# fulliu/lc

Measured on AMD Instinct MI355X. Metric: poses/sec (cov-loss fwd+bwd + weighted PnP), B=256 N=64, 1/2/4/8 MI355X, higher is better.
Workload: dtype f64; 1 GPU; configs[1]: synthetic B=256 N=64 2D-3D correspondences per GPU, HIP weighted-PnP + cov-loss; global_batch=256, n_points=64, launch=graph_region, launch_agreed_by_all_ranks=True

## Files before the change

### lc_amd/csrc/lc_common.h

```cpp
#pragma once
#include <hip/hip_runtime.h>

#include "shared/lc_shared.h"

namespace lc {

typedef float lc_v4f_t __attribute__((ext_vector_type(4)));
__device__ __forceinline__ void store_stream4(float* q, float a, float b, float c, float d) {
    lc_v4f_t r = {a, b, c, d};
    __builtin_nontemporal_store(r, reinterpret_cast<lc_v4f_t*>(q));
}


__device__ __forceinline__ double fast_rcp(double x) {
    const double y = __builtin_amdgcn_rcp(x);
    const double e = __builtin_fma(-x, y, 1.0);
    return __builtin_fma(y, e, y);
}

__device__ __forceinline__ void fast_sqrt_rsqrt(double x, double& s, double& rs) {
    const double r0 = __builtin_amdgcn_rsq(x);
    const double g = x * r0, h = 0.5 * r0;
    const double rr = __builtin_fma(-h, g, 0.5);
    const double g1 = __builtin_fma(g, rr, g), h1 = __builtin_fma(h, rr, h);
    s = x == 0.0 ? 0.0 : g1;
    rs = x == 0.0 ? r0 : 2.0 * h1;
}
__device__ __forceinline__ double fast_sqrt(double x) {
    double s, rs;
    fast_sqrt_rsqrt(x, s, rs);
    return s;
}

__device__ __forceinline__ void wave_sync() {
    __builtin_amdgcn_fence(__ATOMIC_RELEASE, "wavefront");
    __builtin_amdgcn_wave_barrier();
    __builtin_amdgcn_fence(__ATOMIC_ACQUIRE, "wavefront");
}

constexpr int block_sum_lds_doubles(int K) { return K * 68 + K; }
__device__ __forceinline__ int block_sum_open(int lane) {
    wave_sync();
    return lane + 2 * (lane >> 5);
}
template <int ROW = 68>
__device__ __forceinline__ void block_sum_put(double* lds, int pos, int k, double v) { lds[k * ROW + pos] = v; }

__device__ __forceinline__ double block_sum_segment(const double2* row) {
    double2 a[8];
#pragma unroll
    for (int i = 0; i < 8; ++i) a[i] = row[i];
#pragma unroll
    for (int i = 0; i < 8; ++i) {
        const double2 t = row[8 + i];
        a[i].x += t.x;
        a[i].y += t.y;
    }
#pragma unroll
    for (int st = 4; st >= 1; st >>= 1) {
#pragma unroll
        for (int i = 0; i < st; ++i) { a[i].x += a[i + st].x; a[i].y += a[i + st].y; }
    }
    return a[0].x + a[0].y;
}
__device__ __forceinline__ double block_sum_segment_component(const double* d) {
    double a[8];
#pragma unroll
    for (int i = 0; i < 8; ++i) a[i] = d[2 * i];
#pragma unroll
    for (int i = 0; i < 8; ++i) a[i] += d[16 + 2 * i];
#pragma unroll
    for (int st = 4; st >= 1; st >>= 1) {
#pragma unroll
        for (int i = 0; i < st; ++i) a[i] += a[i + st];
    }
    return a[0];
}

template <int K>
__device__ __forceinline__ void block_sum_close(double (&v)[K], double* lds, int lane) {
    static_assert(K <= 32, "two segments per entry, one lane each");
    wave_sync();
    double s = 0;
    if (lane < 2 * K) s = block_sum_segment(reinterpret_cast<const double2*>(lds + (lane / 2) * 68 + 34 * (lane % 2)));
    s += dpp_mov_f64<kDppQuadXor1>(s, s);
    double* tot = lds + K * 68;
    if (lane < 2 * K && (lane % 2) == 0) tot[lane / 2] = s;
    wave_sync();
#pragma unroll
    for (int k = 0; k < K; ++k) v[k] = tot[k];
}

template <class T>
__device__ __forceinline__ void xcd_store(T* q, T v) { __hip_atomic_store(q, v, __ATOMIC_RELAXED, __HIP_MEMORY_SCOPE_AGENT); }
template <class T>
__device__ __forceinline__ T xcd_load(const T* q) { return __hip_atomic_load(q, __ATOMIC_RELAXED, __HIP_MEMORY_SCOPE_AGENT); }
__device__ __forceinline__ void xcd_stores_done() { asm volatile("s_waitcnt vmcnt(0)" ::: "memory"); }

constexpr int kArrivalShards = 16, kArrivalStride = 32;
constexpr int kArrivalWords = (1 + kArrivalShards) * kArrivalStride;
__device__ __forceinline__ bool arrive_is_last(unsigned* words, unsigned block, unsigned blocks) {
    const unsigned shards = blocks < (unsigned)kArrivalShards ? blocks : (unsigned)kArrivalShards;
    const unsigned g = block % shards, members = (blocks - g + shards - 1) / shards;
    if (__hip_atomic_fetch_add(words + (1 + g) * kArrivalStride, 1u, __ATOMIC_RELAXED, __HIP_MEMORY_SCOPE_AGENT) != members - 1) return false;
    return __hip_atomic_fetch_add(words, 1u, __ATOMIC_RELAXED, __HIP_MEMORY_SCOPE_AGENT) == shards - 1;
}
__device__ __forceinline__ void arrival_reset(unsigned* words, int tid) {
    if (tid <= kArrivalShards) xcd_store(words + tid * kArrivalStride, 0u);
}

constexpr int kTeamRowDoubles = 66;
static_assert(kTeamRowDoubles >= 66 && kTeamRowDoubles % 4 == 2, "a row holds two padded segments; rows of one wave fall on different banks");
constexpr int sum_team2_lds_doubles(int K) { return K * kTeamRowDoubles + 2 * K; }
template <int K, int W>
__device__ __forceinline__ void block_sum_team2(double (&v)[K], double* lds, int lane, int& phase) {
    static_assert(K % 2 == 0 && K <= 32 && (W == 0 || W == 1), "an even number of entries dealt to two waves");
    wave_sync();
    double s = 0;
    const int comp = lane & 1, seg = (lane >> 1) & 1, entry = 2 * (lane >> 2) + W;
    if (lane < 2 * K) s = block_sum_segment_component(lds + entry * kTeamRowDoubles + 34 * seg + comp);
    s += dpp_mov_f64<kDppQuadXor1>(s, s);
    s += dpp_mov_f64<kDppQuadXor2>(s, s);
    double* tot = lds + K * kTeamRowDoubles + K * phase;
    phase ^= 1;
    if (lane < 2 * K && (lane % 4) == 0) tot[entry] = s;
    __syncthreads();
#pragma unroll
    for (int k = 0; k < K; ++k) v[k] = tot[k];
}

template <int K>
__device__ __forceinline__ void block_sum_waves4(double (&v)[K], double* lds, int tid, int& phase) {
    static_assert(K <= 32, "one reduce-scatter of 32");
    const int lane = tid & 63, wave = tid >> 6;
    double w[32];
#pragma unroll
    for (int k = 0; k < 32; ++k) w[k] = k < K ? v[k] : 0.0;
    wave_reduce_scatter16<32>(w, lane);
    double* part = lds;
    double* tot = lds + 128 + 32 * phase;
    phase ^= 1;
    if ((lane & 3) == 0) *reinterpret_cast<double2*>(part + 32 * wave + scatter16_base(lane, 2)) = make_double2(w[0], w[1]);
    __syncthreads();
    if (tid < 32) tot[tid] = ((part[tid] + part[32 + tid]) + part[64 + tid]) + part[96 + tid];
    __syncthreads();
#pragma unroll
    for (int k = 0; k < K; ++k) v[k] = tot[k];
}

constexpr int kSplitMaxParts = 8;
#ifndef LC_SPLIT_WAIT_US
#define LC_SPLIT_WAIT_US 2000
#endif
constexpr unsigned long long kSplitWaitTicks = 100ull * LC_SPLIT_WAIT_US;
__device__ __forceinline__ bool split_wait_expired(int polls, unsigned long long& t0) {
    if ((polls & 15) != 15) return false;
    const unsigned long long now = __builtin_amdgcn_s_memrealtime();
    if (t0 == 0) { t0 = now; return false; }
    return now - t0 > kSplitWaitTicks;
}
constexpr int kSplitRowWords = 64;
constexpr size_t kSplitPoseBytes = 2 * kSplitMaxParts * kSplitRowWords * sizeof(unsigned long long) + 128;
constexpr int kSplitLdsDoubles = 128 + 64 + 2;
constexpr int kSplitSerialLdsDoubles = 128 + 32 * kSplitMaxParts + 32;
struct SplitSum {
    unsigned long long* exch;
    unsigned* epoch;
    int G, part;
    unsigned base;
    unsigned seq;
    bool timed_out;
};
__device__ __forceinline__ unsigned* split_tail(void* region, size_t region_bytes) {
    return reinterpret_cast<unsigned*>(static_cast<char*>(region) + region_bytes - 128);
}
__device__ __forceinline__ SplitSum split_sum_enter(void* pose_region, int G, int part) {
    unsigned* epoch = split_tail(pose_region, kSplitPoseBytes);
    return SplitSum{reinterpret_cast<unsigned long long*>(pose_region), epoch, G, part, xcd_load(epoch), 0u, false};
}
__device__ __forceinline__ void split_sum_leave(const SplitSum& sx) {
    if (sx.timed_out) xcd_store(sx.epoch + 1, 1u);
    else if (sx.part == 0 && sx.seq > 0) xcd_store(sx.epoch, sx.base + sx.seq);
}
__device__ __forceinline__ bool split_rescue_enter(void* region, size_t region_bytes, bool redo, int tid, int threads) {
    unsigned* tail = split_tail(region, region_bytes);
    const bool dirty = xcd_load(tail + 1) != 0u;
    if (!dirty && !redo) return false;
    __syncthreads();
    if (dirty) {
        unsigned long long* w = static_cast<unsigned long long*>(region);
        for (size_t i = tid; i < (region_bytes - 128) / 8; i += threads) xcd_store(w + i, 0ull);
        if (tid < 2) xcd_store(tail + tid, 0u);
    }
    if (redo && tid == 0) xcd_store(tail + 2, xcd_load(tail + 2) + 1u);
    return redo;
}

template <int K>
__device__ __forceinline__ void block_sum_split(double (&v)[K], double* lds, int tid, int& phase, SplitSum& sx) {
    static_assert(K <= 32, "one reduce-scatter of 32");
    const int lane = tid & 63, wave = tid >> 6;
    double w[32];
#pragma unroll
    for (int k = 0; k < 32; ++k) w[k] = k < K ? v[k] : 0.0;
    wave_reduce_scatter16<32>(w, lane);
    double* part = lds;
    double* tot = lds + 128 + 32 * phase;
    int* arrived_ok = reinterpret_cast<int*>(lds + 192);
    phase ^= 1;
    if (sx.timed_out) {
#pragma unroll
        for (int k = 0; k < K; ++k) v[k] = 0.0;
        return;
    }
    if ((lane & 3) == 0) *reinterpret_cast<double2*>(part + 32 * wave + scatter16_base(lane, 2)) = make_double2(w[0], w[1]);
    __syncthreads();
    if (tid < 32) {
        const unsigned long long ticket = (unsigned long long)(sx.base + sx.seq + 1u) << 32;
        unsigned long long* rows = sx.exch + (size_t)(sx.seq & 1u) * (kSplitMaxParts * kSplitRowWords) + 2 * tid;
        {
            const unsigned long long bits = __builtin_bit_cast(unsigned long long, ((part[tid] + part[32 + tid]) + part[64 + tid]) + part[96 + tid]);
            unsigned long long* mine = rows + sx.part * kSplitRowWords;
            xcd_store(mine, ticket | (bits & 0xFFFFFFFFull));
            xcd_store(mine + 1, ticket | (bits >> 32));
        }
        unsigned long long lo[kSplitMaxParts], hi[kSplitMaxParts];
        bool ok = true;
        unsigned long long t0 = 0;
        for (int polls = 0;; ++polls) {
#pragma unroll
            for (int g = 0; g < kSplitMaxParts; ++g)
                if (g < sx.G) {
                    lo[g] = xcd_load(rows + g * kSplitRowWords);
                    hi[g] = xcd_load(rows + g * kSplitRowWords + 1);
                }
            unsigned long long late = 0;
#pragma unroll
            for (int g = 0; g < kSplitMaxParts; ++g)
                if (g < sx.G) late |= ((lo[g] ^ ticket) | (hi[g] ^ ticket)) >> 32;
            if (late == 0) break;
            if (split_wait_expired(polls, t0)) { ok = false; break; }
            __builtin_amdgcn_s_sleep(1);
        }
        double s = 0.0;
#pragma unroll
        for (int g = 0; g < kSplitMaxParts; ++g)
            if (g < sx.G) s += __builtin_bit_cast(double, (hi[g] << 32) | (lo[g] & 0xFFFFFFFFull));
        tot[tid] = s;
        if (!ok) *arrived_ok = 0;
    }
    __syncthreads();
    if (!*arrived_ok) sx.timed_out = true;
#pragma unroll
    for (int k = 0; k < K; ++k) v[k] = tot[k];
    ++sx.seq;
}

template <int K>
__device__ __forceinline__ void block_sum_parts_serial(double (&v)[K], double* lds, int tid, int g, int G) {
    static_assert(K <= 32, "one reduce-scatter of 32");
    const int lane = tid & 63, wave = tid >> 6;
    double w[32];
#pragma unroll
    for (int k = 0; k < 32; ++k) w[k] = k < K ? v[k] : 0.0;
    wave_reduce_scatter16<32>(w, lane);
    double* part = lds;
    double* rows = lds + 128;
    double* tot = lds + 128 + 32 * kSplitMaxParts;
    if ((lane & 3) == 0) *reinterpret_cast<double2*>(part + 32 * wave + scatter16_base(lane, 2)) = make_double2(w[0], w[1]);
    __syncthreads();
    if (tid < 32) {
        rows[32 * g + tid] = ((part[tid] + part[32 + tid]) + part[64 + tid]) + part[96 + tid];
        if (g == G - 1) {
            double s = 0.0;
            for (int h = 0; h < G; ++h) s += rows[32 * h + tid];
            tot[tid] = s;
        }
    }
    __syncthreads();
    if (g == G - 1) {
#pragma unroll
        for (int k = 0; k < K; ++k) v[k] = tot[k];
    }
}

__device__ __forceinline__ double horner_step(double p, double z, double c) {
    double r;
    asm("v_fma_f64 %0, %1, %2, %3" : "=v"(r) : "v"(p), "v"(z), "v"(c));
    return r;
}

#ifndef LC_SINCOS_FALLBACK_CALL
#define LC_SINCOS_FALLBACK_CALL 0
#endif
#if LC_SINCOS_FALLBACK_CALL
static __device__ __attribute__((noinline, cold)) double2 sincos_full_range(double x) {
    double s, c;
    sincos(x, &s, &c);
    return make_double2(s, c);
}
#endif
static __device__ __forceinline__ void sincos_small(double x, double& s, double& c) {
#if LC_SINCOS_FALLBACK_CALL
    if (__builtin_expect(!(x < 1.0e4), 0)) {
        const double2 sc = sincos_full_range(x);
        s = sc.x;
        c = sc.y;
        return;
    }
#else
    if (!(x < 1.0e4)) {
        sincos(x, &s, &c);
        return;
    }
#endif
    const double kf = __builtin_rint(x * 0.63661977236758134308);
    const int q = (int)kf;
    double r = __builtin_fma(-kf, 1.57079632673412561417e+00, x);
    r = __builtin_fma(-kf, 6.07710050650619224932e-11, r);
    r = __builtin_fma(-kf, 2.02226624879595063154e-21, r);
    const double z = r * r;
    double ps = horner_step(1.58969099521155010221e-10, z, -2.50507602534068634195e-08);
    ps = horner_step(ps, z, 2.75573137070700676789e-06);
    ps = horner_step(ps, z, -1.98412698298579493134e-04);
    ps = horner_step(ps, z, 8.33333333332248946124e-03);
    ps = horner_step(ps, z, -1.66666666666666324348e-01);
    const double sr = __builtin_fma(ps * z, r, r);
    double pc = horner_step(-1.13596475577881948265e-11, z, 2.08757232129817482790e-09);
    pc = horner_step(pc, z, -2.75573143513906633035e-07);
    pc = horner_step(pc, z, 2.48015872894767294178e-05);
    pc = horner_step(pc, z, -1.38888888888741095749e-03);
    pc = horner_step(pc, z, 4.16666666666666019037e-02);
    const double cr = __builtin_fma(pc * z, z, __builtin_fma(-0.5, z, 1.0));
    const double ss = (q & 1) ? cr : sr, cc = (q & 1) ? sr : cr;
    s = (q & 2) ? -ss : ss;
    c = ((q + 1) & 2) ? -cc : cc;
}

__device__ __forceinline__ double atan_ratio_pos(double s, double c) {
    const bool swap = s > c;
    const double a = swap ? c : s, b = swap ? s : c;
    double t = a * fast_rcp(b);
#pragma unroll
    for (int k = 0; k < 2; ++k) {
        const double h = fast_sqrt(__builtin_fma(t, t, 1.0));
        t = t * fast_rcp(1.0 + h);
    }
    const double w = t * t;
    double p = horner_step(-1.0 / 21.0, w, 1.0 / 19.0);
    p = horner_step(p, w, -1.0 / 17.0);
    p = horner_step(p, w, 1.0 / 15.0);
    p = horner_step(p, w, -1.0 / 13.0);
    p = horner_step(p, w, 1.0 / 11.0);
    p = horner_step(p, w, -1.0 / 9.0);
    p = horner_step(p, w, 1.0 / 7.0);
    p = horner_step(p, w, -1.0 / 5.0);
    p = horner_step(p, w, 1.0 / 3.0);
    const double at = 4.0 * __builtin_fma(-(p * w), t, t);
    return swap ? 1.57079632679489661923 - at : at;
}

__device__ __forceinline__ bool uniform(bool c) { return __builtin_amdgcn_ballot_w64(c) != 0ull; }

}
```

### lc_amd/csrc/lc_pnp_body.h

```cpp
#pragma once
#include <cfloat>

#include "lc_common.h"
#include "lc_kernels.h"

#ifdef LC_STAMPS
#define LC_PSTAMP_DECL unsigned long long pst_[8] = {0, 0, 0, 0, 0, 0, 0, 0}, pt0_ = 0, pt1_ = 0
#define LC_PSTAMP_BEGIN()                                                                 \
    do {                                                                                  \
        __builtin_amdgcn_sched_barrier(0);                                                \
        asm volatile("s_memtime %0\n\ts_waitcnt lgkmcnt(0)" : "=s"(pt0_)::"memory");      \
        __builtin_amdgcn_sched_barrier(0);                                                \
    } while (0)
#define LC_PSTAMP(i)                                                                      \
    do {                                                                                  \
        __builtin_amdgcn_sched_barrier(0);                                                \
        asm volatile("s_memtime %0\n\ts_waitcnt lgkmcnt(0)" : "=s"(pt1_)::"memory");      \
        __builtin_amdgcn_sched_barrier(0);                                                \
        pst_[i] += pt1_ - pt0_;                                                           \
        pt0_ = pt1_;                                                                      \
    } while (0)
#else
#define LC_PSTAMP_DECL
#define LC_PSTAMP_BEGIN() do {} while (0)
#define LC_PSTAMP(i) do {} while (0)
#endif

#ifndef LC_PNP_TEAM2
#define LC_PNP_TEAM2 1
#endif

namespace lc {
namespace pnp {

template <int NW>
constexpr int kPnpLdsDoubles = [] { static_assert(NW == 1, "the four-wave kernels: kPnpWideReservedLdsDoubles"); return block_sum_lds_doubles(28); }();
constexpr int kPnpTeamLdsDoubles = sum_team2_lds_doubles(28);
constexpr int kPnpWideReservedLdsDoubles = 28 * 68 * 4 + 28;
static_assert(kPnpWideReservedLdsDoubles == 7644 && kPnpWideReservedLdsDoubles >= 128 + 64, "reserved size kept; block_sum_waves4 fits");

struct Point {
    double X[3];
    double u, v;
    double a, b, c;
};

struct Rot {
    double R[9];
    double Jr[9];
};

__device__ __forceinline__ void make_rot(const double aa[3], Rot& o) {
    const double x = aa[0], y = aa[1], z = aa[2];
    const double th2 = x * x + y * y + z * z;
    const bool small = !(th2 > DBL_EPSILON);
    double th, ith;
    fast_sqrt_rsqrt(th2, th, ith);
    double s, c;
    sincos_small(th, s, c);
    const double ith2 = ith * ith;
    const double A = small ? 1.0 : s * ith;
    const double B = small ? 0.0 : (1.0 - c) * ith2;
    const double C = small ? 0.0 : (th - s) * ith2 * ith;
    const double cd = small ? 1.0 : c;
    o.R[0] = cd + B * x * x;    o.R[1] = B * x * y - A * z; o.R[2] = B * x * z + A * y;
    o.R[3] = B * x * y + A * z; o.R[4] = cd + B * y * y;    o.R[5] = B * y * z - A * x;
    o.R[6] = B * x * z - A * y; o.R[7] = B * y * z + A * x; o.R[8] = cd + B * z * z;
    const double d = 1.0 - C * th2;
    o.Jr[0] = d + C * x * x;     o.Jr[1] = C * x * y + B * z; o.Jr[2] = C * x * z - B * y;
    o.Jr[3] = C * x * y - B * z; o.Jr[4] = d + C * y * y;     o.Jr[5] = C * y * z + B * x;
    o.Jr[6] = C * x * z + B * y; o.Jr[7] = C * y * z - B * x; o.Jr[8] = d + C * z * z;
}

template <bool FIRST, bool STREAM = false, int PAR = -1>
__device__ __forceinline__ void accumulate_point(const Point& pt, const Rot& rt, const double t[3], const double k[6],
                                                 const double (&sc)[6], double (&acc)[28], double* lds = nullptr, int pos = 0) {
    double rx[3], q[3];
#pragma unroll
    for (int d = 0; d < 3; ++d) {
        rx[d] = rt.R[3 * d] * pt.X[0] + rt.R[3 * d + 1] * pt.X[1] + rt.R[3 * d + 2] * pt.X[2];
        q[d] = rx[d] + t[d];
    }
    const double iz = fast_rcp(q[2]);
    const double up = (q[0] * k[0] + q[1] * k[1]) * iz, vp = (q[0] * k[3] + q[1] * k[4]) * iz;
    const double du = up - pt.u, dv = vp - pt.v;
    const double r[2] = {du * pt.a + dv * pt.b, dv * pt.c};
    const double dup[3] = {k[0] * iz, k[1] * iz, -up * iz};
    const double dvp[3] = {k[3] * iz, k[4] * iz, -vp * iz};
    double J[2][6];
#pragma unroll
    for (int m = 0; m < 3; ++m) {
        J[0][3 + m] = pt.a * dup[m] + pt.b * dvp[m];
        J[1][3 + m] = pt.c * dvp[m];
    }
#pragma unroll
    for (int rr = 0; rr < 2; ++rr) {
        double cr[3];
        cr[0] = rx[1] * J[rr][5] - rx[2] * J[rr][4];
        cr[1] = rx[2] * J[rr][3] - rx[0] * J[rr][5];
        cr[2] = rx[0] * J[rr][4] - rx[1] * J[rr][3];
#pragma unroll
        for (int m = 0; m < 3; ++m) J[rr][m] = (rt.Jr[3 * m] * cr[0] + rt.Jr[3 * m + 1] * cr[1] + rt.Jr[3 * m + 2] * cr[2]) * sc[m];
#pragma unroll
        for (int m = 0; m < 3; ++m) J[rr][3 + m] *= sc[3 + m];
    }
    static_assert(PAR < 0 || STREAM, "entries are dealt by parity where they go to their LDS slots");
    constexpr auto mine = [](int k) { return PAR < 0 || (k & 1) == PAR; };
    constexpr int kRow = PAR < 0 ? 68 : kTeamRowDoubles;
#pragma unroll
    for (int i = 0; i < 6; ++i) {
#pragma unroll
        for (int j = i; j < 6; ++j) {
            if (mine(tri6(i, j))) {
                const double v = __builtin_fma(J[0][i], J[0][j], J[1][i] * J[1][j]);
                if constexpr (STREAM) block_sum_put<kRow>(lds, pos, tri6(i, j), v);
                else acc[tri6(i, j)] = FIRST ? v : acc[tri6(i, j)] + v;
            }
        }
        if (mine(21 + i)) {
            const double gi = __builtin_fma(J[0][i], r[0], J[1][i] * r[1]);
            if constexpr (STREAM) block_sum_put<kRow>(lds, pos, 21 + i, gi);
            else acc[21 + i] = FIRST ? gi : acc[21 + i] + gi;
        }
    }
    if (mine(27)) {
        const double ss = __builtin_fma(r[0], r[0], r[1] * r[1]);
        if constexpr (STREAM) block_sum_put<kRow>(lds, pos, 27, ss);
        else acc[27] = FIRST ? ss : acc[27] + ss;
    }
}

__device__ __forceinline__ bool ldlt_solve6(const double (&A)[21], const double (&dg)[6], const double (&rhs)[6], double (&y)[6]) {
    double L[6][6], Ld[6][6], id[6];
    bool ok = true;
#pragma unroll
    for (int j = 0; j < 6; ++j) {
        double dj = A[tri6(j, j)] + dg[j];
#pragma unroll
        for (int k = 0; k < j; ++k) dj -= L[j][k] * Ld[j][k];
        ok = ok && (dj > 0) && (dj < DBL_MAX);
        id[j] = fast_rcp(dj);
#pragma unroll
        for (int i = j + 1; i < 6; ++i) {
            double v = A[tri6(j, i)];
#pragma unroll
            for (int k = 0; k < j; ++k) v -= L[i][k] * Ld[j][k];
            Ld[i][j] = v;
            L[i][j] = v * id[j];
        }
    }
    double z[6];
#pragma unroll
    for (int i = 0; i < 6; ++i) {
        double v = rhs[i];
#pragma unroll
        for (int k = 0; k < i; ++k) v -= L[i][k] * z[k];
        z[i] = v;
    }
#pragma unroll
    for (int i = 5; i >= 0; --i) {
        double v = z[i] * id[i];
#pragma unroll
        for (int k = i + 1; k < 6; ++k) v -= L[k][i] * y[k];
        y[i] = v;
    }
    return ok;
}

struct RawPoint {
    float X[3];
    float2 u;
    float a, b, c;
};

template <bool OPTS = false>
__device__ __forceinline__ RawPoint load_raw_point(const PnpParams& p, size_t base, int n) {
    RawPoint o;
    const float* X = p.pts3d + (base + n) * 3;
    o.u = *reinterpret_cast<const float2*>(p.pts2d + (base + n) * 2);
    o.X[0] = X[0]; o.X[1] = X[1]; o.X[2] = X[2];
    if (OPTS && p.weight_mask) {
        const float m = p.weight_mask[base + n] ? 1.f : 0.f;
        o.a = m; o.b = 0.f; o.c = m;
    } else if (p.sqrtL) {
        const float4 L = *reinterpret_cast<const float4*>(p.sqrtL + (base + n) * 4);
        o.a = L.x; o.b = L.z; o.c = L.w;
    } else {
        const float2 L = *reinterpret_cast<const float2*>(p.sqrt_diag + (base + n) * 2);
        o.a = L.x; o.b = 0.f; o.c = L.y;
    }
    if constexpr (OPTS) {
        if (p.options & kPnpWeightsAreStd) { o.a = 1.f / (o.a * o.a); o.c = 1.f / (o.c * o.c); }
        if (p.options & kPnpNanToNum) {
            o.u.x = nan_to_num(o.u.x); o.u.y = nan_to_num(o.u.y);
            o.X[0] = nan_to_num(o.X[0]); o.X[1] = nan_to_num(o.X[1]); o.X[2] = nan_to_num(o.X[2]);
            o.a = nan_to_num(o.a); o.b = nan_to_num(o.b); o.c = nan_to_num(o.c);
        }
        if (p.options & kPnpWeightsAreIcov) { o.a = sqrtf(o.a); o.c = sqrtf(o.c); }
    }
    return o;
}
__device__ __forceinline__ Point to_point(const RawPoint& r, const double cam[6]) {
    Point o;
    o.X[0] = r.X[0]; o.X[1] = r.X[1]; o.X[2] = r.X[2];
    o.u = (double)r.u.x - cam[2];
    o.v = (double)r.u.y - cam[5];
    o.a = r.a; o.b = r.b; o.c = r.c;
    return o;
}
template <bool OPTS = false>
__device__ __forceinline__ Point load_point(const PnpParams& p, size_t base, int n, const double cam[6]) {
    return to_point(load_raw_point<OPTS>(p, base, n), cam);
}

__device__ __forceinline__ double max_abs6(const double (&v)[6]) {
    double m = 0;
#pragma unroll
    for (int j = 0; j < 6; ++j) m = fmax(m, fabs(v[j]));
    return m;
}
__device__ __forceinline__ double norm6(const double (&v)[6]) {
    double m = 0;
#pragma unroll
    for (int j = 0; j < 6; ++j) m += v[j] * v[j];
    return fast_sqrt(m);
}

struct FormDefaults {
    static constexpr int NW = 1, PPT = 0, SPLIT = 0, TEAM = -1;
    static constexpr bool REG = true, OPTS = false, TRACE = false, TAIL = false;
};
template <bool O = false>
struct OneWave : FormDefaults { static constexpr bool OPTS = O; };
template <int W>
struct TeamWave : FormDefaults { static constexpr int TEAM = W; };
struct OneWaveTrace : FormDefaults { static constexpr bool TRACE = true; };
struct FourWaves : FormDefaults { static constexpr int NW = 4; };
template <bool O = false>
struct WideReg : FourWaves { static constexpr bool OPTS = O; };
struct WideLoop : FourWaves { static constexpr bool REG = false; };
struct WideTrace : WideLoop { static constexpr bool TRACE = true; };
template <bool O, int P, bool T = false>
struct WideCached : WideLoop { static constexpr bool OPTS = O, TAIL = T; static constexpr int PPT = P; };
template <bool O>
struct SplitPart : WideCached<O, 8, true> { static constexpr int SPLIT = 1; };
template <bool O>
struct SplitRescue : WideLoop { static constexpr bool OPTS = O; static constexpr int SPLIT = 2; };
template <class F>
constexpr bool form_is_legal() {
    static_assert(F::NW == 1 || F::NW == 4, "one wave or four (the team is two one-wave solves side by side)");
    static_assert(!F::REG || (F::PPT == 0 && !F::TAIL && F::SPLIT == 0), "one correspondence per thread: nothing to cache or to walk");
    static_assert(!F::TAIL || F::PPT > 0, "the tail is what lies behind a cached prefix");
    static_assert(F::SPLIT != 1 || (F::NW == 4 && !F::REG && F::PPT > 0 && !F::TRACE), "the split form is the four-wave cached-prefix solve");
    static_assert(F::SPLIT != 2 || (F::NW == 4 && !F::REG && F::PPT == 0 && !F::TRACE), "the rescue form walks memory, part by part");
    static_assert(F::TEAM < 0 || (F::TEAM <= 1 && F::REG && F::NW == 1 && !F::TRACE && !F::OPTS && F::SPLIT == 0), "the team form is the plain one-correspondence-per-lane solve");
    return true;
}

template <class F>
__device__ __forceinline__ void solve_pose(const PnpParams& p, int b, int lane, double* bc, bool store = true, float* handoff = nullptr,
                                           const float* start_override = nullptr, [[maybe_unused]] SplitSum* sx = nullptr) {
    constexpr int NW = F::NW, PPT = F::PPT, SPLIT = F::SPLIT, TEAM = F::TEAM;
    constexpr bool REG = F::REG, OPTS = F::OPTS, TRACE = F::TRACE, TAIL = F::TAIL;
    static_assert(form_is_legal<F>());
    static_assert(NW == 4 || REG, "one wave has one correspondence per lane");
    constexpr int kThreads = kWave * NW;
    const int slot = SPLIT == 1 ? lane + kThreads * sx->part : lane;
    const int stride = SPLIT == 1 ? kThreads * sx->G : kThreads;
#ifdef LC_TRACE_CLOCK
    const unsigned long long t_start_ = __builtin_amdgcn_s_memtime();
#endif
    LC_PSTAMP_DECL;
    LC_PSTAMP_BEGIN();
    const int n = p.counts ? p.counts[b] : p.Nmax;
    const int bk = (OPTS && p.pose_mod > 0) ? b % p.pose_mod : b;
    const float* st_in = start_override ? start_override : (p.start ? p.start + 7 * (size_t)bk : p.states + 7 * (size_t)b);
    const bool filter = OPTS && (p.options & kPnpNanToNum);
    auto fin = [&](float f) { return filter ? nan_to_num(f) : f; };
    if (n < 3) {
        if (lane == 0 && store) {
            p.rets[b] = 1;
            p.result_tr[b] = 1.f;
            if (p.iters) p.iters[b] = 0;
        }
        if (lane < 7) {
            const float v = fin(st_in[lane]);
            if (store && (p.start || start_override || filter)) p.states[7 * (size_t)b + lane] = v;
            if (handoff) handoff[lane] = v;
        }
        return;
    }
    const size_t base = (size_t)b * p.Nmax;
    const bool active = lane < n;
    RawPoint raw;
    if constexpr (REG) raw = load_raw_point<OPTS>(p, base, active ? lane : 0);
    [[maybe_unused]] RawPoint rawc[PPT > 0 ? PPT : 1];
    if constexpr (!REG && PPT > 0) {
#pragma unroll
        for (int k = 0; k < PPT; ++k)
            if (slot + k * stride < n) rawc[k] = load_raw_point<OPTS>(p, base, slot + k * stride);
    }
    double cam[6];
    {
        const float* Kp = p.K + 9 * (size_t)bk;
#pragma unroll
        for (int i = 0; i < 6; ++i) cam[i] = fin(Kp[i]);
    }
    double x[6];
    {
        float stf[7];
#pragma unroll
        for (int i = 0; i < 7; ++i) stf[i] = st_in[i];
        asm volatile("" : "+v"(stf[0]), "+v"(stf[1]), "+v"(stf[2]), "+v"(stf[3]), "+v"(stf[4]), "+v"(stf[5]), "+v"(stf[6]));
        const double q0 = fin(stf[0]), q1 = fin(stf[1]), q2 = fin(stf[2]), q3 = fin(stf[3]);
        const double s2 = q1 * q1 + q2 * q2 + q3 * q3;
        double kk = 2.0;
        if (s2 > 0.0) {
            const double s = fast_sqrt(s2);
            const double half = atan_ratio_pos(s, fabs(q0));
            const double two_theta = 2.0 * ((q0 < 0.0) ? -half : half);
            kk = two_theta / s;
        }
        x[0] = q1 * kk; x[1] = q2 * kk; x[2] = q3 * kk;
        x[3] = fin(stf[4]); x[4] = fin(stf[5]); x[5] = fin(stf[6]);
    }
    LC_PSTAMP(0);
    Point rp;
    if constexpr (REG) {
        rp = to_point(raw, cam);
        if (!active) { rp.a = 0.0; rp.b = 0.0; rp.c = 0.0; }
    }

    [[maybe_unused]] int sum_phase = 0;
    auto evaluate = [&](const double (&xe)[6], const double (&sc)[6], double (&H)[21], double (&g)[6], double& cost) -> bool {
        LC_PSTAMP(1);
        Rot rt;
        make_rot(xe, rt);
        LC_PSTAMP(2);
        const double t[3] = {xe[3], xe[4], xe[5]};
        double acc[28];
        if constexpr (NW == 1 && TEAM < 0) {
            const int pos = block_sum_open(lane);
            accumulate_point<true, true>(rp, rt, t, cam, sc, acc, bc, pos);
            LC_PSTAMP(3);
            block_sum_close<28>(acc, bc, lane);
        } else if constexpr (NW == 1) {
            const int pos = block_sum_open(lane);
            accumulate_point<true, true, TEAM>(rp, rt, t, cam, sc, acc, bc, pos);
            LC_PSTAMP(3);
            block_sum_team2<28, TEAM>(acc, bc, lane, sum_phase);
        } else if constexpr (REG) {
            accumulate_point<true>(rp, rt, t, cam, sc, acc);
            LC_PSTAMP(3);
            block_sum_waves4<28>(acc, bc, lane, sum_phase);
        } else {
#pragma unroll
            for (int i = 0; i < 28; ++i) acc[i] = 0;
            if constexpr (PPT > 0) {
#pragma unroll
                for (int k = 0; k < PPT; ++k)
                    if (slot + k * stride < n) accumulate_point<false>(to_point(rawc[k], cam), rt, t, cam, sc, acc);
                if constexpr (TAIL)
                    for (int i = slot + PPT * stride; i < n; i += stride) accumulate_point<false>(load_point<OPTS>(p, base, i, cam), rt, t, cam, sc, acc);
            } else if constexpr (SPLIT == 2) {
                for (int g = 0; g < sx->G; ++g) {
                    if (g > 0) {
#pragma unroll
                        for (int i = 0; i < 28; ++i) acc[i] = 0;
                    }
                    for (int i = lane + kThreads * g; i < n; i += kThreads * sx->G) accumulate_point<false>(load_point<OPTS>(p, base, i, cam), rt, t, cam, sc, acc);
                    block_sum_parts_serial<28>(acc, bc, lane, g, sx->G);
                }
            } else {
                for (int i = lane; i < n; i += kThreads) accumulate_point<false>(load_point<OPTS>(p, base, i, cam), rt, t, cam, sc, acc);
            }
            LC_PSTAMP(3);
            if constexpr (SPLIT == 2) {}
            else if constexpr (SPLIT == 1) block_sum_split<28>(acc, bc, lane, sum_phase, *sx);
            else block_sum_waves4<28>(acc, bc, lane, sum_phase);
        }
        LC_PSTAMP(4);
#pragma unroll
        for (int i = 0; i < 21; ++i) H[i] = acc[i];
#pragma unroll
        for (int i = 0; i < 6; ++i) g[i] = acc[21 + i];
        const double ss = acc[27];
        cost = 0.5 * ss;
        double chk = ss;
#pragma unroll
        for (int i = 0; i < 6; ++i) chk += H[tri6(i, i)];
        LC_PSTAMP(5);
        if constexpr (SPLIT == 1) {
            if (sx->timed_out) return false;
        }
        return chk <= DBL_MAX;
    };

    const double ftol = p.ftol, ptol = 1e-8, gtol = 1e-10;
    double H[21], g[6], cost;
    double scale[6], iscale[6];
    bool failed;
    {
        const double one[6] = {1, 1, 1, 1, 1, 1};
        failed = !evaluate(x, one, H, g, cost);
#pragma unroll
        for (int j = 0; j < 6; ++j) {
            iscale[j] = 1.0 + fast_sqrt(H[tri6(j, j)]);
            scale[j] = fast_rcp(iscale[j]);
        }
#pragma unroll
        for (int i = 0; i < 6; ++i) {
#pragma unroll
            for (int j = i; j < 6; ++j) H[tri6(i, j)] *= scale[i] * scale[j];
            g[i] *= scale[i];
        }
    }
    auto grad_max = [&](const double (&gs)[6]) {
        double m = 0;
#pragma unroll
        for (int j = 0; j < 6; ++j) m = fmax(m, fabs(gs[j]) * iscale[j]);
        return m;
    };
    double gmax = grad_max(g);
    auto sqnorm6 = [](const double (&v)[6]) {
        double m = 0;
#pragma unroll
        for (int j = 0; j < 6; ++j) m += v[j] * v[j];
        return m;
    };
    double xn2 = sqnorm6(x);
    double radius = 1e4, dfac = 2.0;
    int iter = 0, n_invalid = 0;
    bool converged = false;
    auto trace = [&](int kind, double cost_x, double cost_cand, double mcc, double rho, double step_norm) {
        if constexpr (TRACE) {
            if (lane == 0 && p.trace && iter <= p.trace_rows) {
                double* row = p.trace + ((size_t)b * p.trace_rows + (iter - 1)) * 8;
                row[0] = kind; row[1] = cost_x; row[2] = cost_cand; row[3] = mcc; row[4] = rho; row[5] = step_norm;
                row[6] = radius; row[7] = gmax;
#ifdef LC_TRACE_CLOCK
                row[7] = (double)(__builtin_amdgcn_s_memtime() - t_start_);
#endif
            }
        }
    };

    while (uniform(!failed && !converged)) {
        if (iter >= p.max_iter) break;
        if (uniform(gmax <= gtol || radius <= 1e-32)) { converged = true; break; }
        ++iter;
        double dg[6], y[6];
        const double inv_radius = fast_rcp(radius);
#pragma unroll
        for (int i = 0; i < 6; ++i) dg[i] = fmin(fmax(H[tri6(i, i)], 1e-6), 1e32) * inv_radius;
        LC_PSTAMP(1);
        bool step_ok = ldlt_solve6(H, dg, g, y);
        LC_PSTAMP(6);
        double mcc = 0;
#pragma unroll
        for (int i = 0; i < 6; ++i) mcc += y[i] * (g[i] + dg[i] * y[i]);
        mcc *= 0.5;
        step_ok = step_ok && (mcc > 0.0) && (mcc <= DBL_MAX);
        if (uniform(!step_ok)) {
            if (++n_invalid >= 5) { failed = true; trace(0, cost, 0.0, mcc, 0.0, 0.0); break; }
            radius /= dfac; dfac *= 2.0;
            trace(0, cost, 0.0, mcc, 0.0, 0.0);
            continue;
        }
        n_invalid = 0;
        double xc[6], delta[6];
#pragma unroll
        for (int j = 0; j < 6; ++j) { delta[j] = -y[j] * scale[j]; xc[j] = x[j] + delta[j]; }
        const double sn2 = sqnorm6(delta);
        const bool ptol_in_reach = TRACE || uniform(!(sn2 > 2.0 * ptol * ptol * (xn2 + ptol * ptol)));
        double step_norm = 0.0;
        bool ptol_hit = false;
        if (ptol_in_reach) {
            step_norm = fast_sqrt(sn2);
            ptol_hit = uniform(step_norm <= ptol * (fast_sqrt(xn2) + ptol));
        }
        double cost_c;
        const bool cand_ok = evaluate(xc, scale, H, g, cost_c);
        if constexpr (SPLIT == 1) {
            if (sx->timed_out) { failed = true; break; }
        }
        if (!cand_ok) cost_c = DBL_MAX;
        if (ptol_hit) {
            converged = true; trace(3, cost, cost_c, mcc, 0.0, step_norm); break;
        }
        const double cost_change = cost - cost_c;
        if (uniform(fabs(cost_change) <= ftol * cost)) {
            converged = true; trace(4, cost, cost_c, mcc, cost_change * fast_rcp(mcc), step_norm); break;
        }
        const double rel = cost_change * fast_rcp(mcc);
        if (uniform(rel > 1e-3)) {
#pragma unroll
            for (int j = 0; j < 6; ++j) x[j] = xc[j];
            const double cost_prev = cost;
            cost = cost_c;
            xn2 = sqnorm6(x);
            gmax = grad_max(g);
            const double tq = 2.0 * rel - 1.0;
            radius = fmin(1e16, radius * fast_rcp(fmax(1.0 / 3.0, 1.0 - tq * tq * tq)));
            dfac = 2.0;
            trace(1, cost_prev, cost_c, mcc, rel, step_norm);
        } else {
            radius /= dfac; dfac *= 2.0;
            trace(2, cost, cost_c, mcc, rel, step_norm);
            double cost_again;
            if (!evaluate(x, scale, H, g, cost_again)) { failed = true; break; }
        }
    }
    LC_PSTAMP(1);
#ifdef LC_STAMPS
    if (lane == 0 && store && p.iters) {
        unsigned long long* o = reinterpret_cast<unsigned long long*>(p.iters) + 8 * (size_t)b;
        for (int i = 0; i < 6; ++i) o[i] = pst_[i];
        o[6] = iter;
        o[7] = pst_[6];
    }
#endif
    const bool invalid = failed || !converged;
    if (invalid && lane < 7) {
        const float v = fin(st_in[lane]);
        if (store && (p.start || start_override || filter)) p.states[7 * (size_t)b + lane] = v;
        if (handoff) handoff[lane] = v;
    }
    if (lane == 0) {
        if (store) {
            p.rets[b] = invalid ? 1 : 0;
            if constexpr (SPLIT == 1) {
                if (sx->timed_out) p.rets[b] = kPnpPartNeverArrived;
            }
            p.result_tr[b] = (float)radius;
#ifndef LC_STAMPS
            if (p.iters) p.iters[b] = iter;
#endif
        }
        if (!invalid) {
            float stq[7];
            float* st = stq;
            const double t2 = x[0] * x[0] + x[1] * x[1] + x[2] * x[2];
            double q0 = 1.0, kk = 0.5;
            if (t2 > 0.0) {
                const double th = fast_sqrt(t2), h = 0.5 * th;
                double sh, ch;
                sincos_small(h, sh, ch);
                q0 = ch;
                kk = sh / th;
            }
            st[0] = (float)q0; st[1] = (float)(x[0] * kk); st[2] = (float)(x[1] * kk); st[3] = (float)(x[2] * kk);
            st[4] = (float)x[3]; st[5] = (float)x[4]; st[6] = (float)x[5];
#pragma unroll
            for (int k = 0; k < 7; ++k) {
                if (store) p.states[7 * (size_t)b + k] = stq[k];
                if (handoff) handoff[k] = stq[k];
            }
        }
    }
}

}
}
```

### lc_amd/csrc/shared/lc_shared.h

```cpp
#pragma once
#include <hip/hip_runtime.h>

#include <cfloat>

namespace lc {

constexpr int kWave = 64;

constexpr int kDppQuadXor1 = 0xB1;
constexpr int kDppQuadXor2 = 0x4E;
constexpr int kDppIdentity = 0xE4;
constexpr int kDppRowMirror = 0x140;
constexpr int kDppHalfMirror = 0x141;

template <int CTRL, int BANK_MASK = 0xF>
__device__ __forceinline__ double dpp_mov_f64(double old, double src) {
    const int lo = __builtin_amdgcn_update_dpp(__double2loint(old), __double2loint(src), CTRL, 0xF, BANK_MASK, false);
    const int hi = __builtin_amdgcn_update_dpp(__double2hiint(old), __double2hiint(src), CTRL, 0xF, BANK_MASK, false);
    return __hiloint2double(hi, lo);
}

__device__ __forceinline__ double shfl_f64(double v, int src) {
    const int lo = __shfl(__double2loint(v), src, kWave), hi = __shfl(__double2hiint(v), src, kWave);
    return __hiloint2double(hi, lo);
}

__device__ __forceinline__ double swap32_add(double a, double b) {
    const auto lo = __builtin_amdgcn_permlane32_swap(__double2loint(a), __double2loint(b), false, false);
    const auto hi = __builtin_amdgcn_permlane32_swap(__double2hiint(a), __double2hiint(b), false, false);
    return __hiloint2double(hi[0], lo[0]) + __hiloint2double(hi[1], lo[1]);
}
__device__ __forceinline__ double swap16_add(double a, double b) {
    const auto lo = __builtin_amdgcn_permlane16_swap(__double2loint(a), __double2loint(b), false, false);
    const auto hi = __builtin_amdgcn_permlane16_swap(__double2hiint(a), __double2hiint(b), false, false);
    return __hiloint2double(hi[0], lo[0]) + __hiloint2double(hi[1], lo[1]);
}

template <int CTRL, int BANK_UP>
__device__ __forceinline__ double dpp_exchange_add(double lo, double hi) {
    constexpr int BANK_DOWN = 0xF & ~BANK_UP;
    const double keep = dpp_mov_f64<kDppIdentity, BANK_UP>(lo, hi);
    double recv = dpp_mov_f64<CTRL, BANK_UP>(lo, hi);
    recv = dpp_mov_f64<CTRL, BANK_DOWN>(recv, lo);
    return keep + recv;
}

template <int K>
__device__ __forceinline__ void wave_allreduce(double (&v)[K]) {
#pragma unroll
    for (int i = 0; i < K; ++i) {
        double x = v[i];
        x += dpp_mov_f64<kDppQuadXor1>(x, x);
        x += dpp_mov_f64<kDppQuadXor2>(x, x);
        x += dpp_mov_f64<kDppHalfMirror>(x, x);
        x += dpp_mov_f64<kDppRowMirror>(x, x);
        x = swap16_add(x, x);
        x = swap32_add(x, x);
        v[i] = x;
    }
}

template <int K>
__device__ __forceinline__ void wave_reduce_scatter16(double (&v)[K], int ) {
    static_assert(K % 16 == 0, "K must be a multiple of 16");
    constexpr int R = K / 16;
#pragma unroll
    for (int i = 0; i < K / 2; ++i) v[i] = swap32_add(v[i], v[i + K / 2]);
#pragma unroll
    for (int i = 0; i < K / 4; ++i) v[i] = swap16_add(v[i], v[i + K / 4]);
#pragma unroll
    for (int i = 0; i < K / 8; ++i) v[i] = dpp_exchange_add<kDppRowMirror, 0xC>(v[i], v[i + K / 8]);
#pragma unroll
    for (int i = 0; i < K / 16; ++i) v[i] = dpp_exchange_add<kDppHalfMirror, 0xA>(v[i], v[i + K / 16]);
#pragma unroll
    for (int i = 0; i < R; ++i) {
        v[i] += dpp_mov_f64<kDppQuadXor2>(v[i], v[i]);
        v[i] += dpp_mov_f64<kDppQuadXor1>(v[i], v[i]);
    }
}

__device__ __forceinline__ int scatter16_base(int lane, int R) {
    return R * (((lane >> 5) & 1) * 8 + ((lane >> 4) & 1) * 4 + ((lane >> 3) & 1) * 2 + ((lane >> 2) & 1));
}

__host__ __device__ constexpr int tri6(int i, int j) { return i * 6 - (i * (i - 1)) / 2 + (j - i); }

__device__ __forceinline__ float nan_to_num(float f) { return f != f ? 0.f : fminf(fmaxf(f, -FLT_MAX), FLT_MAX); }

__device__ __forceinline__ void quat_matrix(const double q[4], double two_s, double R[9]) {
    const double r = q[0], i = q[1], j = q[2], k = q[3];
    R[0] = 1 - two_s * (j * j + k * k); R[1] = two_s * (i * j - k * r); R[2] = two_s * (i * k + j * r);
    R[3] = two_s * (i * j + k * r); R[4] = 1 - two_s * (i * i + k * k); R[5] = two_s * (j * k - i * r);
    R[6] = two_s * (i * k - j * r); R[7] = two_s * (j * k + i * r); R[8] = 1 - two_s * (i * i + j * j);
}

}
```

Baseline: 20.79 million poses/s.

## Reduce team-of-two PnP normal equations in registers via wave reduce-scatter

For the two-wave team PnP path, each lane now keeps its 14 parity-dealt normal-equation entries in registers and runs a cross-lane reduce-scatter (permlane swaps and DPP row exchanges) that leaves each sum in LDS order. Only the final per-entry totals are written to a small LDS buffer before one barrier. This replaces streaming every per-point entry into a padded LDS tile followed by segment reads. The aim is less LDS traffic and a smaller LDS footprint, paid for with more register pressure and extra DPP/permlane instructions.

```diff
diff --git a/lc_amd/csrc/lc_common.h b/lc_amd/csrc/lc_common.h
--- a/lc_amd/csrc/lc_common.h
+++ b/lc_amd/csrc/lc_common.h
@@ -124,6 +124,23 @@
     double* tot = lds + K * kTeamRowDoubles + K * phase;
     phase ^= 1;
     if (lane < 2 * K && (lane % 4) == 0) tot[entry] = s;
+    __syncthreads();
+#pragma unroll
+    for (int k = 0; k < K; ++k) v[k] = tot[k];
+}
+
+constexpr int sum_team2_reg_lds_doubles(int K) { return 2 * K; }
+template <int K, int W>
+__device__ __forceinline__ void block_sum_team2_reg(double (&v)[K], double* lds, int lane, int& phase) {
+    static_assert(K % 2 == 0 && K <= 32 && (W == 0 || W == 1), "an even number of entries dealt to two waves");
+    double w[K / 2];
+#pragma unroll
+    for (int i = 0; i < K / 2; ++i) w[i] = v[2 * i + W];
+    const double s = wave_reduce_scatter_lds_order<K / 2>(w, lane);
+    double* tot = lds + K * phase;
+    phase ^= 1;
+    const int entry = reduce_scatter_lds_order_entry<K / 2>((lane >> 1) & 15);
+    if (lane < 32 && (lane & 1) == 0 && entry >= 0) tot[2 * entry + W] = s;
     __syncthreads();
 #pragma unroll
     for (int k = 0; k < K; ++k) v[k] = tot[k];
diff --git a/lc_amd/csrc/lc_pnp_body.h b/lc_amd/csrc/lc_pnp_body.h
--- a/lc_amd/csrc/lc_pnp_body.h
+++ b/lc_amd/csrc/lc_pnp_body.h
@@ -29,13 +29,20 @@
 #ifndef LC_PNP_TEAM2
 #define LC_PNP_TEAM2 1
 #endif
+#ifndef LC_PNP_TEAM_REGSUM
+#define LC_PNP_TEAM_REGSUM 1
+#endif
 
 namespace lc {
 namespace pnp {
 
 template <int NW>
 constexpr int kPnpLdsDoubles = [] { static_assert(NW == 1, "the four-wave kernels: kPnpWideReservedLdsDoubles"); return block_sum_lds_doubles(28); }();
+#if LC_PNP_TEAM_REGSUM
+constexpr int kPnpTeamLdsDoubles = sum_team2_reg_lds_doubles(28);
+#else
 constexpr int kPnpTeamLdsDoubles = sum_team2_lds_doubles(28);
+#endif
 constexpr int kPnpWideReservedLdsDoubles = 28 * 68 * 4 + 28;
 static_assert(kPnpWideReservedLdsDoubles == 7644 && kPnpWideReservedLdsDoubles >= 128 + 64, "reserved size kept; block_sum_waves4 fits");
 
@@ -104,7 +111,7 @@
 #pragma unroll
         for (int m = 0; m < 3; ++m) J[rr][3 + m] *= sc[3 + m];
     }
-    static_assert(PAR < 0 || STREAM, "entries are dealt by parity where they go to their LDS slots");
+    static_assert(PAR < 0 || FIRST, "entries are dealt by parity where a lane owns one point");
     constexpr auto mine = [](int k) { return PAR < 0 || (k & 1) == PAR; };
     constexpr int kRow = PAR < 0 ? 68 : kTeamRowDoubles;
 #pragma unroll
@@ -345,10 +352,16 @@
             LC_PSTAMP(3);
             block_sum_close<28>(acc, bc, lane);
         } else if constexpr (NW == 1) {
+#if LC_PNP_TEAM_REGSUM
+            accumulate_point<true, false, TEAM>(rp, rt, t, cam, sc, acc);
+            LC_PSTAMP(3);
+            block_sum_team2_reg<28, TEAM>(acc, bc, lane, sum_phase);
+#else
             const int pos = block_sum_open(lane);
             accumulate_point<true, true, TEAM>(rp, rt, t, cam, sc, acc, bc, pos);
             LC_PSTAMP(3);
             block_sum_team2<28, TEAM>(acc, bc, lane, sum_phase);
+#endif
         } else if constexpr (REG) {
             accumulate_point<true>(rp, rt, t, cam, sc, acc);
             LC_PSTAMP(3);
diff --git a/lc_amd/csrc/shared/lc_shared.h b/lc_amd/csrc/shared/lc_shared.h
--- a/lc_amd/csrc/shared/lc_shared.h
+++ b/lc_amd/csrc/shared/lc_shared.h
@@ -83,6 +83,51 @@
     return R * (((lane >> 5) & 1) * 8 + ((lane >> 4) & 1) * 4 + ((lane >> 3) & 1) * 2 + ((lane >> 2) & 1));
 }
 
+template <int K>
+__device__ __forceinline__ constexpr int reduce_scatter_lds_order_entry(int slot) {
+    static_assert(K == 14 || K == 16, "16 slots, or 14 with slots 7 and 15 empty");
+    if (K == 16) return slot;
+    return (slot & 7) == 7 ? -1 : slot - (slot >> 3);
+}
+constexpr int kDppRowRor8 = 0x128;
+constexpr int kDppRowShl4 = 0x104;
+constexpr int kDppRowShr4 = 0x114;
+template <int K>
+__device__ __forceinline__ double wave_reduce_scatter_lds_order(const double (&v)[K], int lane) {
+    constexpr auto entry = reduce_scatter_lds_order_entry<K>;
+    static_assert((entry(7) < 0) == (entry(15) < 0), "an empty slot's partner is empty");
+    double w[8];
+#pragma unroll
+    for (int i = 0; i < 8; ++i) {
+        if (entry(i) >= 0) w[i] = swap16_add(v[entry(i)], v[entry(i + 8)]);
+    }
+    const bool up8 = (lane & 8) != 0, up4 = (lane & 4) != 0;
+    auto exchange8 = [up8](double lo, double hi) {
+        const double keep = up8 ? hi : lo;
+        double recv = dpp_mov_f64<kDppRowRor8>(lo, lo);
+        recv = dpp_mov_f64<kDppRowRor8, 0xC>(recv, hi);
+        return keep + recv;
+    };
+    w[0] = exchange8(w[0], w[4]);
+    w[1] = exchange8(w[1], w[5]);
+    w[2] = exchange8(w[2], w[6]);
+    if constexpr (entry(7) >= 0) w[3] = exchange8(w[3], w[7]);
+    else w[3] += dpp_mov_f64<kDppRowRor8>(w[3], w[3]);
+    auto exchange4 = [up4](double lo, double hi) {
+        const double keep = up4 ? hi : lo;
+        double recv = dpp_mov_f64<kDppRowShl4, 0x5>(lo, lo);
+        recv = dpp_mov_f64<kDppRowShr4, 0xA>(recv, hi);
+        return keep + recv;
+    };
+    w[0] = exchange4(w[0], w[2]);
+    w[1] = exchange4(w[1], w[3]);
+    const bool up = (lane & 2) != 0;
+    const double keep = up ? w[1] : w[0], send = up ? w[0] : w[1];
+    double s = keep + dpp_mov_f64<kDppQuadXor2>(send, send);
+    s += dpp_mov_f64<kDppQuadXor1>(s, s);
+    return swap32_add(s, s);
+}
+
 __host__ __device__ constexpr int tri6(int i, int j) { return i * 6 - (i * (i - 1)) / 2 + (j - i); }
 
 __device__ __forceinline__ float nan_to_num(float f) { return f != f ? 0.f : fminf(fmaxf(f, -FLT_MAX), FLT_MAX); }
```

Result: faster. 21.04 million poses/s, median of 6 (+1.2%).
